# Bernat-C/MRI-Diffusion-SuperResolution

Hardware: AMD Instinct MI355X
Metric: MRI slices/sec (50-step DDIM, 256^2, bs=32) (higher is better)
Workload: dtype bf16; 1 GPU; configs[1]: 256x256 1-ch synthetic MRI slices -> 4x32x32 latents, SD-1.5-size UNet (859.5M params, random init) + rank-4 LoRA, 50-step DDIM, bs=32 per GPU; ddim_steps=50, parallelism=slice-sharded x1 (no collective), lora=explicit adapters, down-projection + rank-r update inside the projection GEMMs, tile_table=profiles/r03_tune_cache.tsv, hipgraph=True

## Files before the change

include/mrisr_debug.h:

```cpp
#ifndef MRISR_DEBUG_H
#define MRISR_DEBUG_H
#ifdef __cplusplus
extern "C" {
#endif

void mrisr_debug_force_split(int splitk);
void mrisr_debug_force_tile(int tile);
void mrisr_debug_prefer_tile(int tile);
void mrisr_debug_gemm_flags(int flags);
void mrisr_debug_gemm_stamps(void* dev_buf, int tile);
void mrisr_debug_group_m(int group_m);
void mrisr_debug_op_conv_pad0(int on);
void mrisr_debug_set_tile_eff(int tile, double eff);
void mrisr_debug_set_tuned(const char* key, int tile, int splitk);
void mrisr_debug_gn_fused(int on);

int mrisr_autotune_stats(int* shapes, double* ms);
void mrisr_autotune_release(void);

int mrisr_bench_gemm(int M, int N, int K, int conv, int B, int H, int W, int stride, int ups, int c1, int tile, int splitk,
                     int iters, float* ms_out);

void mrisr_debug_sk_inkernel(int on);

void mrisr_debug_subpix(int min_rows);

void mrisr_debug_temb_table(int on);

void mrisr_debug_mlp_proj(int on);

void mrisr_debug_gn_slabs(int on);

void mrisr_debug_sc_fused(int on);

void mrisr_debug_ff_proj_fused(int on);

void mrisr_debug_xattn_tail(int on);
void mrisr_debug_xattn_tail_stamps(void* dev_buf);

int mrisr_bench_mlp(int M, int hidden, int iters, float* ms_out);

#ifdef __cplusplus
}
#endif
#endif
```

mri-diffusion-superresolution_amd/csrc/capi_ops.hip:

```cpp
#include <algorithm>
#include <cmath>
#include <cstring>
#include <memory>
#include <vector>

#include "api.h"
#include "model.h"
#include "train_ops.h"

using namespace mrisr;

namespace {
struct OpScratch {
    std::vector<std::unique_ptr<DevBuf>> bufs;
    void* alloc(size_t bytes, bool zero = false) {
        bufs.emplace_back(new DevBuf());
        if (bufs.back()->reserve(bytes ? bytes : 1, zero)) return nullptr;
        return bufs.back()->p;
    }
};
template <typename T>
int op_gemm_run(OpScratch& sc, hipStream_t st, GemmArgs& g) {
    return gemm_run<T>(g, st, false, [&sc](size_t n) { return sc.alloc(n); });
}
// ... 598 lines not shown
    a.x0 = x->data; a.c0 = (int)x->shape[1];
    if (x2) { a.x1 = x2->data; a.c1 = (int)x2->shape[1]; }
    a.B = (int)x->shape[0]; a.HW = (int)(x->shape[2] * x->shape[3]); a.groups = groups; a.eps = eps;
    a.gamma = gamma_dev; a.beta = beta_dev; a.silu = silu; a.y = y->data;
    a.nsplit = groupnorm_nsplit(a.B, a.HW);
    DevBuf part;
    TRY(part.reserve((size_t)a.B * a.nsplit * groups * 2 * sizeof(float), false));
    a.partial = static_cast<float*>(part.p);
    int rc = x->dtype == MRISR_F32 ? launch_groupnorm<float>(a, st) : launch_groupnorm<bf16>(a, st);
    if (rc) return rc;
    MRISR_CHECK_HIP(hipStreamSynchronize(st));
    return 0;
    API_END
}

int mrisr_op_layernorm(const mrisr_tensor* x, const float* gamma_dev, const float* beta_dev, float eps,
                       mrisr_tensor* y, void* stream) {
    API_BEGIN
    TRY(op_dtype_ok(x));
    MRISR_REQUIRE(x->ndim == 2 && y && y->dtype == x->dtype, "rows in/out");
    hipStream_t st = (hipStream_t)stream;
    const int M = (int)x->shape[0], C = (int)x->shape[1];
    return x->dtype == MRISR_F32 ? launch_layernorm<float>(x->data, y->data, gamma_dev, beta_dev, M, C, eps, st)
                                 : launch_layernorm<bf16>(x->data, y->data, gamma_dev, beta_dev, M, C, eps, st);
    API_END
}

int mrisr_op_attention(const mrisr_tensor* q, const mrisr_tensor* k, const mrisr_tensor* v, int heads, int flash,
                       mrisr_tensor* out, void* stream) {
    API_BEGIN
// ... 617 lines not shown
```

mri-diffusion-superresolution_amd/csrc/common.h:

```cpp
#pragma once
#include <hip/hip_runtime.h>
#include <stdint.h>
#include <string>

#include "lora_hr.h"

namespace mrisr {

typedef __bf16 bf16;
typedef __attribute__((ext_vector_type(8))) __bf16 bf16x8;
typedef __attribute__((ext_vector_type(4))) __bf16 bf16x4;
typedef __attribute__((ext_vector_type(4))) float f32x4;
typedef __attribute__((ext_vector_type(16))) float f32x16;

enum DType : int { DT_F32 = 0, DT_BF16 = 1, DT_F16 = 2, DT_I64 = 3 };

template <typename T> struct TypeTag;
template <> struct TypeTag<float> { static constexpr int id = DT_F32; };
template <> struct TypeTag<bf16> { static constexpr int id = DT_BF16; };

__device__ __forceinline__ float to_f32(float x) { return x; }
__device__ __forceinline__ float to_f32(bf16 x) { return (float)x; }
template <typename T> __device__ __forceinline__ T from_f32(float x);
template <> __device__ __forceinline__ float from_f32<float>(float x) { return x; }
// ... 172 lines not shown
    int nsplit = 1;
};
extern int g_plan_salt;
int groupnorm_nsplit(int B, int HW);
struct GnSlabSrc {
    const float* partial = nullptr;
    int splitk = 1;
    float alpha = 1.f;
    const float* bias = nullptr;
    const float* rowvec = nullptr;
    int rowvec_ld = 0, rowvec_div = 1;
    const void* resid = nullptr;
    int ldr = 0;
    void* raw_out = nullptr;
};
bool groupnorm_slabs_ok(int C, int groups, int HW);
int launch_groupnorm_slabs(const GroupNormArgs& a, const GnSlabSrc& s, hipStream_t st);
bool gn_fused_geometry(int c0, int c1, int groups, int HW, int* slab, int* slots, int* rl, int* nv, int ve = 8);
template <typename T> int launch_groupnorm(const GroupNormArgs& a, hipStream_t st);
template <typename T>
int launch_layernorm(const void* x, void* y, const float* gamma, const float* beta, int M, int C, float eps,
                     hipStream_t st);
template <typename T>
int launch_softmax_rows(const float* s, int ld, void* p, int ldp, long long rows, int nk, hipStream_t st);

struct GroupNormBwdArgs {
    const void* x0 = nullptr;
    const void* x1 = nullptr;
    int c0 = 0, c1 = 0, B = 0, HW = 0, groups = 32;
    float eps = 1e-5f;
    const float* gamma = nullptr;
// ... 204 lines not shown
```

mri-diffusion-superresolution_amd/csrc/norm.hip:

```cpp
#include "common.h"
#include "prof.h"

namespace mrisr {

template <typename T> struct Vec;
template <> struct Vec<bf16> {
    static constexpr int N = 8;
    typedef bf16x8 type;
};
template <> struct Vec<float> {
    static constexpr int N = 4;
    typedef f32x4 type;
};

template <typename T, int VPT>
__global__ __launch_bounds__(256) void gn_stats_kernel(const GroupNormArgs a, int slots, int RL) {
    constexpr int VE = Vec<T>::N;
    typedef typename Vec<T>::type vec_t;
    extern __shared__ float sm[];
    const int C = a.c0 + a.c1;
    const int b = blockIdx.y, sp = blockIdx.x;
    const int tid = threadIdx.x;
    const int slot = tid % slots, rl = tid / slots;
    const int rows_per = (a.HW + a.nsplit - 1) / a.nsplit;
// ... 118 lines not shown
            for (int v = 0; v < VPT; ++v) {
                const int ch = (slot * VPT + v) * VE;
                vec_t o;
#pragma unroll
                for (int e = 0; e < VE; ++e) {
                    float f = (float)xv[u][v][e] * sc[v][e] + sh[v][e];
                    if (a.silu) f = silu_f(f);
                    o[e] = from_f32<T>(f);
                }
                *reinterpret_cast<vec_t*>(y + (size_t)r * C + ch) = o;
            }
        }
    }
}

template <int NVM, int VE, bool SLAB = false, int NT = 256>
__global__ __launch_bounds__(NT) void gn_fused_kernel(const GroupNormArgs a, int slab, int slots, int RL, int nslab, int xcd_map, const GnSlabSrc ss = GnSlabSrc()) {
    typedef bf16 T;
    typedef __attribute__((ext_vector_type(VE))) __bf16 vec_t;
    __shared__ float part[NT * 16];
    __shared__ float seg[2 * 1280];
    __shared__ double gsum[2 * 80];
    __shared__ float mean_s[80], rstd_s[80];
    const int C = a.c0 + a.c1;
    const int Cg = C / a.groups;
    int b, sl;
    if (xcd_map) {
        const int L = blockIdx.x;
        b = (L & 7) + 8 * (L / (8 * nslab));
        sl = (L >> 3) % nslab;
    } else {
// ... 2 lines not shown
    }
    const int ch0 = sl * slab;
    const int tid = threadIdx.x;
    const int slot = tid % slots, rl = tid / slots;
    const bool active = rl < RL;
    const int ch = ch0 + slot * VE;
    const T* src;
    int ld;
    if (ch < a.c0) { src = reinterpret_cast<const T*>(a.x0) + (size_t)b * a.HW * a.c0 + ch; ld = a.c0; }
    else { src = reinterpret_cast<const T*>(a.x1) + (size_t)b * a.HW * a.c1 + (ch - a.c0); ld = a.c1; }
    vec_t xv[NVM];
    float s1[VE], s2[VE];
#pragma unroll
    for (int e = 0; e < VE; ++e) s1[e] = s2[e] = 0.f;
    if (active) {
        if constexpr (SLAB) {
            typedef __attribute__((ext_vector_type(VE))) float fvec_t;
            const size_t MN = (size_t)a.B * a.HW * C;
            fvec_t bv;
#pragma unroll
            for (int e = 0; e < VE; ++e) bv[e] = 0.f;
            if (ss.bias) bv = *reinterpret_cast<const fvec_t*>(ss.bias + ch);
#pragma unroll
            for (int i = 0; i < NVM; ++i) {
                const int r = rl + i * RL;
                if (r < a.HW) {
                    const size_t mrow = (size_t)b * a.HW + r;
                    const float* pp = ss.partial + mrow * C + ch;
                    fvec_t v;
#pragma unroll
                    for (int e = 0; e < VE; ++e) v[e] = 0.f;
                    for (int sp = 0; sp < ss.splitk; ++sp) {
                        const fvec_t t = *reinterpret_cast<const fvec_t*>(pp + (size_t)sp * MN);
#pragma unroll
                        for (int e = 0; e < VE; ++e) v[e] += t[e];
                    }
#pragma unroll
                    for (int e = 0; e < VE; ++e) v[e] = v[e] * ss.alpha + bv[e];
                    if (ss.rowvec) {
                        const fvec_t t = *reinterpret_cast<const fvec_t*>(ss.rowvec + (mrow / ss.rowvec_div) * ss.rowvec_ld + ch);
#pragma unroll
                        for (int e = 0; e < VE; ++e) v[e] += t[e];
                    }
                    if (ss.resid) {
                        const vec_t t = *reinterpret_cast<const vec_t*>(reinterpret_cast<const T*>(ss.resid) + mrow * ss.ldr + ch);
#pragma unroll
                        for (int e = 0; e < VE; ++e) v[e] += (float)t[e];
                    }
#pragma unroll
                    for (int e = 0; e < VE; ++e) xv[i][e] = (bf16)v[e];
                    if (ss.raw_out) *reinterpret_cast<vec_t*>(reinterpret_cast<T*>(ss.raw_out) + mrow * C + ch) = xv[i];
                }
            }
        } else {
#pragma unroll
        for (int i = 0; i < NVM; ++i) {
            const int r = rl + i * RL;
            if (r < a.HW) xv[i] = *reinterpret_cast<const vec_t*>(src + (size_t)r * ld);
        }
        }
#pragma unroll
        for (int i = 0; i < NVM; ++i) {
            if (rl + i * RL < a.HW) {
#pragma unroll
                for (int e = 0; e < VE; ++e) {
                    const float f = (float)xv[i][e];
                    s1[e] += f;
// ... 202 lines not shown
    if (rows_per_block < RL) rows_per_block = RL;
    bx = (a.HW + rows_per_block - 1) / rows_per_block;
    ProfScope ps2(prof_intern(n2), 0.0, 2.0 * act_bytes, st);
    switch (vpt) {
        case 1: hipLaunchKernelGGL((gn_apply_kernel<T, 1>), dim3(bx, a.B), dim3(256), 0, st, a, slots, RL, rows_per_block); break;
        case 2: hipLaunchKernelGGL((gn_apply_kernel<T, 2>), dim3(bx, a.B), dim3(256), 0, st, a, slots, RL, rows_per_block); break;
        case 3: hipLaunchKernelGGL((gn_apply_kernel<T, 3>), dim3(bx, a.B), dim3(256), 0, st, a, slots, RL, rows_per_block); break;
        default: hipLaunchKernelGGL((gn_apply_kernel<T, 4>), dim3(bx, a.B), dim3(256), 0, st, a, slots, RL, rows_per_block); break;
    }
    MRISR_CHECK_HIP(hipGetLastError());
    return 0;
}

static int g_gn_slabs = -1;
extern "C" void mrisr_debug_gn_slabs(int on) { g_gn_slabs = on; ++g_plan_salt; }
static bool gn_slabs_geometry(int C, int groups, int HW, int B, int* ve, int* slab, int* slots, int* rl, int* nv) {
    if (!gn_fused_geometry(C, 0, groups, HW, slab, slots, rl, nv, 8)) return false;
    *ve = 8;
    int s4 = 0, sl4 = 0, rl4 = 0, nv4 = 0;
    if (B * (C / *slab) < 512 && gn_fused_geometry(C, 0, groups, HW, &s4, &sl4, &rl4, &nv4, 4) && C / s4 > C / *slab) {
        *ve = 4; *slab = s4; *slots = sl4; *rl = rl4; *nv = nv4;
    }
    return *nv <= 8;
}
bool groupnorm_slabs_ok(int C, int groups, int HW) {
    static const int env = [] { const char* e = getenv("MRISR_GN_SLABS"); return e ? atoi(e) : 1; }();
    if (g_gn_slabs < 0 ? !env : !g_gn_slabs) return false;
    if (C % groups || groups > 64 || C % 8) return false;
    int ve, slab, slots, rl, nv;
    return gn_slabs_geometry(C, groups, HW, 32, &ve, &slab, &slots, &rl, &nv);
}
int launch_groupnorm_slabs(const GroupNormArgs& a, const GnSlabSrc& s, hipStream_t st) {
    const int C = a.c0;
    MRISR_REQUIRE(a.c1 == 0 && a.x1 == nullptr && C % a.groups == 0 && a.groups <= 64 && C % 8 == 0, "GroupNorm from slabs: one source, whole groups");
    MRISR_REQUIRE(s.partial && s.splitk >= 1 && a.partial != nullptr && a.nsplit >= 1 && (!s.rowvec || s.rowvec_div >= 1) && (!s.resid || s.ldr % 8 == 0), "GroupNorm from slabs: operands");
    int ve, slab, slots, rl, nv;
    MRISR_REQUIRE(gn_slabs_geometry(C, a.groups, a.HW, a.B, &ve, &slab, &slots, &rl, &nv), "GroupNorm from slabs: geometry (groupnorm_slabs_ok)");
    const int nslab = C / slab;
    const int xmap = (a.B % 8) == 0 ? 1 : 0;
    std::string nf = "groupnorm_from_slabs";
    if (prof_enabled() && prof_shapes()) {
        char buf[96];
        snprintf(buf, sizeof(buf), " B=%d HW=%d C=%d s=%d", a.B, a.HW, C, s.splitk);
        nf += buf;
    }
    const double act_bytes = (double)a.B * a.HW * C * 2.0;
    ProfScope ps(prof_intern(nf), 0.0, act_bytes * (2.0 * s.splitk + 1.0 + (s.raw_out ? 1.0 : 0.0) + (s.resid ? 1.0 : 0.0)), st);
    const dim3 fg(a.B * nslab);
#define GNS_GO(NV, VEV) hipLaunchKernelGGL((gn_fused_kernel<NV, VEV, true>), fg, dim3(256), 0, st, a, slab, slots, rl, nslab, xmap, s)
    if (ve == 8) { if (nv <= 2) GNS_GO(2, 8); else if (nv <= 4) GNS_GO(4, 8); else GNS_GO(8, 8); }
    else { if (nv <= 2) GNS_GO(2, 4); else if (nv <= 4) GNS_GO(4, 4); else GNS_GO(8, 4); }
#undef GNS_GO
    MRISR_CHECK_HIP(hipGetLastError());
    return 0;
}

__device__ __forceinline__ float wave_sum(float v) {
#pragma unroll
    for (int o = 32; o > 0; o >>= 1) v += __shfl_xor(v, o);
    return v;
}
__device__ __forceinline__ float wave_max(float v) {
#pragma unroll
    for (int o = 32; o > 0; o >>= 1) v = fmaxf(v, __shfl_xor(v, o));
    return v;
}

// ... 241 lines not shown
```

mri-diffusion-superresolution_amd/csrc/runner.h:

```cpp
#pragma once
#include <climits>
#include <cmath>
#include <cstdlib>

#include "api.h"
#include "gemm_args.h"
#include "model.h"

namespace mrisr {

extern int g_subpix_override;

inline bool fuse_ln() {
    static int v = -1;
    if (v < 0) { const char* e = getenv("MRISR_FUSE_LN"); v = (e && e[0] == '0') ? 0 : 1; }
    return v == 1;
}
inline bool lora_in_kernel() {
    static int v = -1;
    if (v < 0) { const char* e = getenv("MRISR_LORA_INKERNEL"); v = (e && e[0] == '0') ? 0 : 1; }
    return v == 1;
}

template <typename T>
// ... 90 lines not shown
        *out = new_act(x.B, x.H, x.W, cw.cout);
        if (!out->p) return 7;
        GroupNormArgs a;
        a.x0 = nullptr; a.c0 = cw.cout; a.B = x.B; a.HW = x.H * x.W; a.groups = m.cfg.norm_num_groups; a.eps = eps;
        a.gamma = nw.g; a.beta = nw.b; a.silu = silu ? 1 : 0; a.y = out->p;
        a.nsplit = groupnorm_nsplit(a.B, a.HW);
        a.partial = static_cast<float*>(alloc((size_t)a.B * a.nsplit * a.groups * 2 * sizeof(float)));
        TRY(gemm_alloc_partial(g, arena_alloc()));
        if (!a.partial) return 7;
        if (dry) return 0;
        g.defer_reduce = 1;
        TRY(launch_gemm<T>(g, st));
        GnSlabSrc ss;
        ss.partial = g.partial; ss.splitk = g.splitk; ss.alpha = g.alpha; ss.bias = g.bias; ss.rowvec = g.rowvec; ss.rowvec_ld = g.rowvec_ld;
        ss.rowvec_div = g.rowvec_div; ss.resid = g.resid; ss.ldr = g.ldr; ss.raw_out = h.p;
        return launch_groupnorm_slabs(a, ss, st);
    }

    static int subpix_min_rows() {
        static const int v = [] { const char* e = getenv("MRISR_SUBPIX"); return e ? atoi(e) : 2048; }();
        return g_subpix_override >= 0 ? g_subpix_override : v;
    }
    int upsample_conv(const Act& x, const Level& lv, Act* out) {
        const int minr = subpix_min_rows();
        if (!(sizeof(T) == 2 && lv.up_sp && !m.keep && minr > 0 && (long long)x.rows() >= minr))
            return conv3(x, nullptr, lv.up, 1, 1, nullptr, 0, 1, nullptr, ACT_NONE, out);
        const ConvW& cw = lv.up;
        MRISR_REQUIRE(cw.cin == x.C, "upsampler weight mismatch");
        *out = new_act(x.B, 2 * x.H, 2 * x.W, cw.cout);
        if (!out->p) return 7;
// ... 93 lines not shown
        TRY(gn(t->h, nullptr, r.n2, true, m.cfg.norm_eps, &t->hn, &t->p2, &t->ns2));
        Act res = x;
        if (r.has_sc) {
            GemmArgs g = resnet_shortcut_args(x, x1, r.sc.w, r.sc.b, r.cin, r.cout, o.p);
            TRY(run_gemm(g));
            res = o;
        } else {
            MRISR_REQUIRE(!x1, "concat input requires a shortcut conv");
        }
        if (r.c2.r) TRY(conv_lora_z(t->hn, r.c2, &t->z2));
        GemmArgs g = resnet_conv2_args(t->hn.p, x.B, x.H, x.W, r.cout, r.c2.w, r.c2.b, res.p, o.p);
        if (t->z2) ga_lora_epilogue(g, r.c2, t->z2);
        return run_gemm(g);
    }

    int resnet(const ResW& r, const Act& x, const Act* x1, Act* out, const NormW* next = nullptr, float next_eps = 0.f, Act* next_out = nullptr) {
        Act o = new_act(x.B, x.H, x.W, r.cout);
        if (!o.p) return 7;
        if (next_out) next_out->p = nullptr;
        if (r.c1.r || r.c2.r) {
            const size_t mk0 = m.arena.mark();
            ResTape t;
            TRY(resnet_literal(r, x, x1, o, &t));
            if (!m.keep) m.arena.release(mk0);
            *out = o;
            return 0;
        }
        GemmArgs g2;
        bool fuse2 = false;
        GroupNormArgs a2;
        GemmArgs gt = resnet_conv2_args(kUnallocated, x.B, x.H, x.W, r.cout, r.c2sc, r.b2sc, nullptr, o.p, r.cin, &x, x1);
        const bool sc_tail = sizeof(T) == 2 && !m.keep && r.has_sc && r.c2sc && sc_fused_enabled() && x.C + (x1 ? x1->C : 0) == r.cin && gemm_sc_tail_ok(gt);
        if (next && next_out && sizeof(T) == 2 && !m.keep && next->c == r.cout && groupnorm_slabs_ok(r.cout, m.cfg.norm_num_groups, x.H * x.W)) {
            g2 = sc_tail ? gt
                         : resnet_conv2_args(kUnallocated, x.B, x.H, x.W, r.cout, r.c2.w, r.c2.b, kUnallocated, kUnallocated);
            TRY(gemm_choose(g2, true));
            fuse2 = g2.splitk > 1;
            if (fuse2) {
                *next_out = new_act(x.B, x.H, x.W, r.cout);
                a2.nsplit = groupnorm_nsplit(x.B, x.H * x.W);
                a2.partial = static_cast<float*>(alloc((size_t)x.B * a2.nsplit * m.cfg.norm_num_groups * 2 * sizeof(float)));
                if (!next_out->p || !a2.partial) return 7;
            }
        }
        const size_t mk = m.arena.mark();
        Act xn, h, hn;
        TRY(gn(x, x1, r.n1, true, m.cfg.norm_eps, &xn));
        const int div = m.t_scalar ? INT_MAX : x.H * x.W;
        TRY(conv3_gn(xn, nullptr, r.c1, m.tproj_out + r.temb_off, m.tproj_total, div, nullptr, r.n2, true, m.cfg.norm_eps, nullptr, &hn));
        Act res = x;
        if (sc_tail) {
            res.p = nullptr;
        } else if (r.has_sc) {
            GemmArgs g = resnet_shortcut_args(x, x1, r.sc.w, r.sc.b, r.cin, r.cout, o.p);
            MRISR_REQUIRE(r.sc.R == 0, "shortcut has no LoRA");
            TRY(run_gemm(g));
            res = o;
        } else {
            MRISR_REQUIRE(!x1, "concat input requires a shortcut conv");
        }
        if (fuse2) {
            g2.a0 = hn.p; g2.resid = res.p; g2.out = o.p;
            TRY(gemm_alloc_partial(g2, arena_alloc()));
            if (!dry) {
                g2.defer_reduce = 1;
                TRY(launch_gemm<T>(g2, st));
                a2.x0 = nullptr; a2.c0 = r.cout; a2.B = x.B; a2.HW = x.H * x.W; a2.groups = m.cfg.norm_num_groups; a2.eps = next_eps;
                a2.gamma = next->g; a2.beta = next->b; a2.silu = 0; a2.y = next_out->p;
                GnSlabSrc ss;
                ss.partial = g2.partial; ss.splitk = g2.splitk; ss.alpha = g2.alpha; ss.bias = g2.bias; ss.resid = res.p; ss.ldr = r.cout; ss.raw_out = o.p;
                TRY(launch_groupnorm_slabs(a2, ss, st));
            }
        } else if (sc_tail) {
            gt.a0 = hn.p;
            TRY(run_gemm(gt));
        } else {
            GemmArgs g = resnet_conv2_args(hn.p, x.B, x.H, x.W, r.cout, r.c2.w, r.c2.b, res.p, o.p);
            TRY(run_gemm(g));
        }
        if (!m.keep) m.arena.release(mk);
        *out = o;
        return 0;
    }
// ... 231 lines not shown
            MRISR_CHECK_HIP(hipMemcpyAsync(t.data, a.p, a.numel() * sizeof(T), hipMemcpyDeviceToDevice, st));
            return 0;
        }
        return launch_nhwc_to_nchw<T>(a.p, t.data, t.dtype, a.B, a.C, a.H, a.W, scale, st);
    }
    int add_external(Act& x, const mrisr_tensor& t) {
        const size_t mk = m.arena.mark();
        Act r;
        TRY(import_act(t, &r, false));
        MRISR_REQUIRE(r.B == x.B && r.C == x.C && r.H == x.H && r.W == x.W, "residual shape mismatch");
        if (!dry) TRY(launch_add_inplace<T>(x.p, r.p, (long long)x.numel(), st));
        if (!m.keep) m.arena.release(mk);
        return 0;
    }

    int encoder(Act x, const mrisr_tensor* intrablock, int n_intra, std::vector<Act>* skips, Act* out, int last_skip = -1) {
        skips->push_back(x);
        int ib = 0;
        auto done = [&] { return last_skip >= 0 && (int)skips->size() > last_skip; };
        for (int i = 0; i < m.cfg.num_levels && !done(); ++i) {
            Level& lv = m.down[i];
            const bool has_attn = !lv.xf.empty();
            const int block_last = (int)skips->size() - 1 + (int)lv.res.size() + (lv.has_down ? 1 : 0);
            for (size_t j = 0; j < lv.res.size() && !done(); ++j) {
                Act y, xn_next;
                xn_next.p = nullptr;
                if (has_attn) TRY(resnet(lv.res[j], x, nullptr, &y, &lv.xf[j].norm, 1e-6f, &xn_next));
                else TRY(resnet(lv.res[j], x, nullptr, &y));
                x = y;
                if (has_attn) {
                    TRY(transformer(lv.xf[j], x, &y, &xn_next));
                    x = y;
                    if (j + 1 == lv.res.size() && ib < n_intra) TRY(add_external(x, intrablock[ib++]));
                }
                skips->push_back(x);
            }
            if (lv.has_down && !done()) {
                Act y;
                TRY(conv3(x, nullptr, lv.down, 2, 0, nullptr, 0, 1, nullptr, ACT_NONE, &y));
                x = y;
                skips->push_back(x);
            }
            if (!has_attn && ib < n_intra && (last_skip < 0 || last_skip >= block_last)) {
                TRY(add_external(x, intrablock[ib++]));
            }
        }
        *out = x;
        return 0;
    }
    int mid(Act x, Act* out) {
        Act y, xn_next;
        xn_next.p = nullptr;
        TRY(resnet(m.mid_r0, x, nullptr, &y, &m.mid_xf.norm, 1e-6f, &xn_next));
        x = y;
        TRY(transformer(m.mid_xf, x, &y, &xn_next));
        x = y;
        TRY(resnet(m.mid_r1, x, nullptr, &y));
        *out = y;
        return 0;
    }

    int set_context(const mrisr_tensor& ehs) {
        MRISR_REQUIRE(ehs.ndim == 3 && ehs.shape[2] == m.cfg.cross_attention_dim, "encoder_hidden_states shape");
        MRISR_REQUIRE((int)ehs.shape[0] == m.ws_B && (int)ehs.shape[1] == m.ctx_len, "context shape vs planned workspace");
        if (!dry) TRY(launch_nchw_to_nhwc<T>(ehs.data, ehs.dtype, m.ctx_rows, m.ws_B * m.ctx_len, m.cfg.cross_attention_dim, 1, 1, st));
        auto each = [&](XfW& x) -> int { return project_context(x, m.head_buf_for_C(x.C)); };
        for (auto& lv : m.down) for (auto& x : lv.xf) TRY(each(x));
        TRY(each(m.mid_xf));
// ... 16 lines not shown
        m.arena.reset();
        const int B = (int)sample.shape[0];
        const bool store = fc.mode == CACHE_STORE, use = fc.mode == CACHE_USE;
        const int q0 = m.num_skips() - 1 - fc.depth;
        if (store || use) {
            MRISR_REQUIRE(q0 >= 0 && fc.depth >= 1 && fc.p, "feature cache: depth 1 .. num_skips - 1 and a buffer");
            MRISR_REQUIRE(n_down == 0 && !mid_res, "a feature cache together with ControlNet residuals is not supported");
        }
        if (ehs) TRY(set_context(*ehs));
        MRISR_REQUIRE(dry || m.ctx_valid, "no encoder_hidden_states given and none cached");
        TRY(time_embed(t_dev, t_scalar, B));
        Act s, x;
        TRY(import_act(sample, &s, false));
        TRY(direct(s, m.conv_in, 1, ACT_NONE, nullptr, &x));
        std::vector<Act> skips;
        TRY(encoder(x, intrablock, n_intra, &skips, &x, use ? fc.depth : -1));
        if (n_down > 0) {
            MRISR_REQUIRE(n_down == (int)skips.size(), "down_block_additional_residuals count");
            for (int k = 0; k < n_down; ++k) {
                if (skips[k].p == x.p) {
                    Act c = new_act(x.B, x.H, x.W, x.C);
                    if (!c.p) return 7;
                    if (!dry) MRISR_CHECK_HIP(hipMemcpyAsync(c.p, x.p, x.numel() * sizeof(T), hipMemcpyDeviceToDevice, st));
                    skips[k] = c;
                }
                TRY(add_external(skips[k], down_res[k]));
            }
        }
        if (!use) TRY(mid(x, &x));
        if (mid_res) TRY(add_external(x, *mid_res));
        int q = 0;
        for (int i = 0; i < m.cfg.num_levels; ++i) {
            Level& lv = m.up[i];
            for (size_t j = 0; j < lv.res.size(); ++j, ++q) {
                if (use && q < q0) continue;
                if ((store || use) && q == q0) {
                    int64_t cs[4];
                    TRY(m.cache_shape(fc.depth, B, (int)sample.shape[2], (int)sample.shape[3], cs));
                    if (store) {
                        MRISR_REQUIRE(x.B == cs[0] && x.C == cs[1] && x.H == cs[2] && x.W == cs[3], "feature cache shape");
                        if (!dry) MRISR_CHECK_HIP(hipMemcpyAsync(fc.p, x.p, x.numel() * sizeof(T), hipMemcpyDeviceToDevice, st));
                    } else {
                        x.p = fc.p; x.B = (int)cs[0]; x.C = (int)cs[1]; x.H = (int)cs[2]; x.W = (int)cs[3];
                    }
// ... 46 lines not shown
    int controlnet_forward(const mrisr_tensor& sample, const long long* t_dev, int t_scalar, const mrisr_tensor* ehs,
                           const mrisr_tensor* cond, float scale, mrisr_tensor* down_out, int n_down,
                           mrisr_tensor* mid_out) {
        m.arena.reset();
        const int B = (int)sample.shape[0];
        if (ehs) TRY(set_context(*ehs));
        if (cond) TRY(set_cond(*cond));
        MRISR_REQUIRE(dry || (m.ctx_valid && m.cond_valid), "context / condition image neither given nor cached");
        TRY(time_embed(t_dev, t_scalar, B));
        Act s, x;
        TRY(import_act(sample, &s, false));
        Act ce;
        ce.p = m.cond_emb; ce.B = B; ce.H = s.H; ce.W = s.W; ce.C = m.cfg.block_out_channels[0];
        TRY(direct(s, m.conv_in, 1, ACT_NONE, &ce, &x));
        std::vector<Act> skips;
        TRY(encoder(x, nullptr, 0, &skips, &x));
        TRY(mid(x, &x));
        MRISR_REQUIRE(n_down == (int)skips.size(), "ControlNet output count");
        for (int k = 0; k < n_down; ++k) {
            const size_t mk = m.arena.mark();
            Act o = new_act(skips[k].B, skips[k].H, skips[k].W, skips[k].C);
            if (!o.p) return 7;
            TRY(linear(skips[k].p, (int)skips[k].rows(), skips[k].C, m.cn_down[k], ACT_NONE, nullptr, 0, nullptr, o.p, o.C));
            TRY(export_act(o, down_out[k], scale));
            if (!m.keep) m.arena.release(mk);
        }
        Act o = new_act(x.B, x.H, x.W, x.C);
        if (!o.p) return 7;
        TRY(linear(x.p, (int)x.rows(), x.C, m.cn_mid, ACT_NONE, nullptr, 0, nullptr, o.p, o.C));
        return export_act(o, *mid_out, scale);
    }
};
// ... 3 lines not shown
```

mri-diffusion-superresolution_amd/mrisr/_lib.py:

```python
from __future__ import annotations

import ctypes as C
import os
from typing import Optional, Sequence

import torch

_HERE = os.path.dirname(os.path.abspath(__file__))
LIB_PATH = os.path.join(os.path.dirname(_HERE), "csrc", "libmrisr.so")

MRISR_F32, MRISR_BF16, MRISR_F16, MRISR_I64 = 0, 1, 2, 3
MRISR_NCHW, MRISR_NHWC = 0, 1
STEP_DDIM, STEP_RESSHIFT, STEP_DDPM, STEP_UNIPC, STEP_DPMSOLVERPP = 0, 1, 2, 3, 4
ACT_NONE, ACT_RELU, ACT_SILU, ACT_GEGLU = 0, 1, 2, 3
TILE_WINDOWS = {"uniform": 0, "gaussian": 1}

_DT = {torch.float32: MRISR_F32, torch.bfloat16: MRISR_BF16, torch.float16: MRISR_F16, torch.int64: MRISR_I64}


class Tensor(C.Structure):
    _fields_ = [("data", C.c_void_p), ("dtype", C.c_int32), ("layout", C.c_int32), ("ndim", C.c_int32),
                ("shape", C.c_int64 * 4)]


# ... 72 lines not shown
        L.mrisr_sampler_destroy.restype = None
        L.mrisr_sampler_set_clip.argtypes = [C.c_void_p, C.c_float]
        L.mrisr_sampler_set_guidance.argtypes = [C.c_void_p, C.c_float, C.c_float]
        L.mrisr_op_guided_step.argtypes = [C.c_int, C.c_void_p, C.c_void_p, C.c_void_p, C.c_void_p, C.c_void_p, C.c_void_p, C.c_float,
                                           C.c_float, C.c_float, C.c_void_p]
        L.mrisr_sampler_set_cache.argtypes = [C.c_void_p, C.c_int, C.c_int]
        L.mrisr_unet_cache_shape.argtypes = [C.c_void_p, C.c_int, C.c_int, C.c_int, C.c_int, C.c_void_p]
        L.mrisr_unet_forward_cached.argtypes = [C.c_void_p, C.c_void_p, C.c_void_p, C.c_void_p, C.c_void_p, C.c_int, C.c_int, C.c_int,
                                                C.c_void_p, C.c_void_p, C.c_void_p]
        L.mrisr_sampler_set_solver.argtypes = [C.c_void_p, C.c_int, C.c_int, C.c_int, C.c_void_p, C.c_int]
        L.mrisr_op_multistep_step.argtypes = [C.c_int, C.c_void_p, C.c_void_p, C.c_void_p, C.c_void_p, C.c_void_p, C.c_void_p, C.c_void_p,
                                              C.c_int, C.c_int, C.c_float, C.c_float, C.c_void_p]
        P, I, F, Q = C.c_void_p, C.c_int, C.c_float, C.c_int64
        L.mrisr_op_groupnorm_bwd.argtypes = [I, P, I, P, I, I, I, P, P, I, F, I, P, P, I, P, I, P, P, P]
        L.mrisr_op_layernorm_bwd.argtypes = [I, P, P, P, P, I, I, F, I, P, P, P]
        L.mrisr_op_geglu.argtypes = [I, I, P, P, P, Q, I, P]
        L.mrisr_op_pointwise_bwd.argtypes = [I, I, P, P, P, P, Q, I, I, I, I, I, I, I, P]
        L.mrisr_op_lora_wgrad.argtypes = [I, P, I, P, I, I, I, I, I, I, I, P, P, P, F, P]
        L.mrisr_op_lora_wgrad_geglu.argtypes = [I, P, I, P, I, I, I, I, P, F, P]
        L.mrisr_op_lora_wgrad_hr.argtypes = [I, P, I, P, I, I, I, I, I, I, I, P, P, P, F, I, P]
        L.mrisr_op_dora_scale.argtypes = [I, P, P, P, P, F, P, P, I, I, I, I, I, I, P]
        L.mrisr_op_dora_mag_grad.argtypes = [I, P, I, P, I, P, I, P, P, P, I, I, I, P]
        L.mrisr_model_set_dora.argtypes = [P, I]
        L.mrisr_op_transpose.argtypes = [I, P, P, I, I, I, I, Q, Q, I, I, P]
        L.mrisr_op_softmax_bwd.argtypes = [I, P, P, P, I, Q, I, F, P]
        L.mrisr_op_small_dense_bwd.argtypes = [I, I, P, I, P, I, I, I, I, I, P, I, P, P, I, P]
        L.mrisr_op_conv_wgrad.argtypes = [I, P, I, I, I, I, P, I, I, I, I, I, P, P, I, I, I, P]
        L.mrisr_op_conv_dgrad.argtypes = [I, P, I, I, I, I, P, I, I, P, I, P]
        L.mrisr_op_conv_lora_down.argtypes = [I, P, I, I, I, I, P, I, P, I, P]
        L.mrisr_op_conv_lora_dgrad.argtypes = [I, P, I, I, I, I, P, I, P, I, P]
# ... 88 lines not shown
```

mri-diffusion-superresolution_amd/mrisr/ops.py:

```python
from __future__ import annotations

import ctypes as C
from typing import Optional

import torch

from . import _lib as L


def _nhwc(x: torch.Tensor):
    buf = x.permute(0, 2, 3, 1).contiguous()
    return buf, L.as_tensor(buf, L.MRISR_NHWC, shape=x.shape)


def _f32(x: Optional[torch.Tensor]):
    return None if x is None else C.c_void_p(x.detach().to(torch.float32).contiguous().data_ptr())


def conv3x3(x, weight, bias=None, x2=None, stride=1, upsample=False, act=L.ACT_NONE, splitk=0, tile=0, subpix=False):
    xb, tx = _nhwc(x)
    t2 = None
    if x2 is not None:
        x2b, t2 = _nhwc(x2)
    w = weight.detach().to(torch.float32).contiguous()
# ... 144 lines not shown
    ctot = x.shape[1]
    if x2 is not None:
        x2b, t2 = _nhwc(x2)
        ctot += x2.shape[1]
    g = gamma.detach().to(torch.float32).contiguous()
    b = beta.detach().to(torch.float32).contiguous()
    B, _, H, W = x.shape
    yb = torch.empty((B, H, W, ctot), dtype=x.dtype, device=x.device)
    ty = L.as_tensor(yb, L.MRISR_NHWC, shape=(B, ctot, H, W))
    L.check(L.lib().mrisr_op_groupnorm(C.byref(tx), C.byref(t2) if t2 else None, C.c_void_p(g.data_ptr()),
                                       C.c_void_p(b.data_ptr()), groups, C.c_float(eps), 1 if silu else 0,
                                       C.byref(ty), L.stream_ptr()))
    return yb.permute(0, 3, 1, 2)


def layernorm(x, gamma, beta, eps=1e-5):
    x = x.contiguous()
    g = gamma.detach().to(torch.float32).contiguous()
    b = beta.detach().to(torch.float32).contiguous()
    y = torch.empty_like(x)
    tx, ty = L.as_tensor(x), L.as_tensor(y)
    L.check(L.lib().mrisr_op_layernorm(C.byref(tx), C.c_void_p(g.data_ptr()), C.c_void_p(b.data_ptr()), C.c_float(eps),
                                       C.byref(ty), L.stream_ptr()))
    torch.cuda.current_stream().synchronize()
    return y


def attention(q, k, v, heads, flash=True, fp8=False):
    q, k, v = q.contiguous(), k.contiguous(), v.contiguous()
    out = torch.empty_like(q)
# ... 179 lines not shown
```

Baseline: 72.54 slices/s.

## Fuse split-K reduce with next GroupNorm in encoder downsample and resnet chains

Adds a conv3_down path in which the stride-2 downsample conv defers its split-K reduction into the GroupNorm-from-slabs kernel of the next resnet's first norm (with SiLU). Resnet outputs in non-attention encoder levels now also produce the next block's normalized input, which is passed forward as a precomputed `pre` activation so the following resnet skips its own GroupNorm. The slab kernel gains a split-K-specialized variant that batches partial-slab loads across rows, and it accepts a second concatenated source. This removes separate reduce and norm passes over activations, at the cost of more template instantiations and more complex encoder control flow.

```diff
diff --git a/include/mrisr_debug.h b/include/mrisr_debug.h
--- a/include/mrisr_debug.h
+++ b/include/mrisr_debug.h
@@ -31,6 +31,10 @@
 
 void mrisr_debug_gn_slabs(int on);
 
+int mrisr_op_groupnorm_slabs(const float* slabs, int splitk, int B, int HW, int C, const float* bias, const float* rowvec, int rowvec_ld,
+                             int rowvec_div, const void* resid, int ldr, const void* x1, int c1, const float* gamma_dev, const float* beta_dev,
+                             int groups, float eps, int silu, int merged, void* y, void* raw, int* merged_out, void* stream);
+
 void mrisr_debug_sc_fused(int on);
 
 void mrisr_debug_ff_proj_fused(int on);
diff --git a/mri-diffusion-superresolution_amd/csrc/capi_ops.hip b/mri-diffusion-superresolution_amd/csrc/capi_ops.hip
--- a/mri-diffusion-superresolution_amd/csrc/capi_ops.hip
+++ b/mri-diffusion-superresolution_amd/csrc/capi_ops.hip
@@ -636,6 +636,43 @@
     API_END
 }
 
+int mrisr_op_groupnorm_slabs(const float* slabs, int splitk, int B, int HW, int C, const float* bias, const float* rowvec, int rowvec_ld,
+                             int rowvec_div, const void* resid, int ldr, const void* x1, int c1, const float* gamma_dev, const float* beta_dev,
+                             int groups, float eps, int silu, int merged, void* y, void* raw, int* merged_out, void* stream) {
+    API_BEGIN
+    MRISR_REQUIRE(slabs && splitk >= 1 && B >= 1 && HW >= 1 && C >= 8 && C % 8 == 0 && gamma_dev && beta_dev && y, "GroupNorm from slabs: operands");
+    MRISR_REQUIRE((c1 == 0) == (x1 == nullptr) && c1 % 8 == 0 && (C + c1) % groups == 0 && groups <= 64, "GroupNorm from slabs: second source, groups");
+    MRISR_REQUIRE((!rowvec || (rowvec_div >= 1 && rowvec_ld >= C)) && (!resid || (ldr >= C && ldr % 8 == 0)), "GroupNorm from slabs: time row / residual pitch");
+    hipStream_t st = (hipStream_t)stream;
+    GroupNormArgs a;
+    a.B = B; a.HW = HW; a.groups = groups; a.eps = eps; a.gamma = gamma_dev; a.beta = beta_dev; a.silu = silu; a.y = y;
+    a.nsplit = groupnorm_nsplit(B, HW);
+    DevBuf part, tmp;
+    TRY(part.reserve((size_t)B * a.nsplit * groups * 2 * sizeof(float), false));
+    a.partial = static_cast<float*>(part.p);
+    const bool go = merged && groupnorm_slabs_ok(C, groups, HW, c1, B);
+    if (merged_out) *merged_out = go ? 1 : 0;
+    if (go) {
+        a.x0 = nullptr; a.c0 = C; a.x1 = x1; a.c1 = c1;
+        GnSlabSrc ss;
+        ss.partial = slabs; ss.splitk = splitk; ss.bias = bias; ss.rowvec = rowvec; ss.rowvec_ld = rowvec_ld; ss.rowvec_div = rowvec_div;
+        ss.resid = resid; ss.ldr = ldr; ss.raw_out = raw;
+        TRY(launch_groupnorm_slabs(a, ss, st));
+    } else {
+        void* h = raw;
+        if (!h) { TRY(tmp.reserve((size_t)B * HW * C * sizeof(bf16), false)); h = tmp.p; }
+        GemmArgs g;
+        g.M = B * HW; g.N = C; g.splitk = splitk; g.partial = const_cast<float*>(slabs); g.bias = bias;
+        ga_rowvec(g, rowvec, rowvec_ld, rowvec_div); ga_resid(g, resid, ldr); ga_out(g, h, C);
+        TRY(launch_splitk_reduce<bf16>(g, st));
+        a.x0 = h; a.c0 = C; a.x1 = x1; a.c1 = c1;
+        TRY(launch_groupnorm<bf16>(a, st));
+    }
+    MRISR_CHECK_HIP(hipStreamSynchronize(st));
+    return 0;
+    API_END
+}
+
 int mrisr_op_layernorm(const mrisr_tensor* x, const float* gamma_dev, const float* beta_dev, float eps,
                        mrisr_tensor* y, void* stream) {
     API_BEGIN
diff --git a/mri-diffusion-superresolution_amd/csrc/common.h b/mri-diffusion-superresolution_amd/csrc/common.h
--- a/mri-diffusion-superresolution_amd/csrc/common.h
+++ b/mri-diffusion-superresolution_amd/csrc/common.h
@@ -210,7 +210,7 @@
     int ldr = 0;
     void* raw_out = nullptr;
 };
-bool groupnorm_slabs_ok(int C, int groups, int HW);
+bool groupnorm_slabs_ok(int C, int groups, int HW, int c1 = 0, int B = 32);
 int launch_groupnorm_slabs(const GroupNormArgs& a, const GnSlabSrc& s, hipStream_t st);
 bool gn_fused_geometry(int c0, int c1, int groups, int HW, int* slab, int* slots, int* rl, int* nv, int ve = 8);
 template <typename T> int launch_groupnorm(const GroupNormArgs& a, hipStream_t st);
diff --git a/mri-diffusion-superresolution_amd/csrc/norm.hip b/mri-diffusion-superresolution_amd/csrc/norm.hip
--- a/mri-diffusion-superresolution_amd/csrc/norm.hip
+++ b/mri-diffusion-superresolution_amd/csrc/norm.hip
@@ -156,7 +156,7 @@
     }
 }
 
-template <int NVM, int VE, bool SLAB = false, int NT = 256>
+template <int NVM, int VE, bool SLAB = false, int NT = 256, int SK = 0>
 __global__ __launch_bounds__(NT) void gn_fused_kernel(const GroupNormArgs a, int slab, int slots, int RL, int nslab, int xcd_map, const GnSlabSrc ss = GnSlabSrc()) {
     typedef bf16 T;
     typedef __attribute__((ext_vector_type(VE))) __bf16 vec_t;
@@ -189,19 +189,83 @@
 #pragma unroll
     for (int e = 0; e < VE; ++e) s1[e] = s2[e] = 0.f;
     if (active) {
-        if constexpr (SLAB) {
+        if (SLAB && ch0 < a.c0) {
             typedef __attribute__((ext_vector_type(VE))) float fvec_t;
-            const size_t MN = (size_t)a.B * a.HW * C;
+            const int Cs = a.c0;
+            const size_t MN = (size_t)a.B * a.HW * Cs;
             fvec_t bv;
 #pragma unroll
             for (int e = 0; e < VE; ++e) bv[e] = 0.f;
             if (ss.bias) bv = *reinterpret_cast<const fvec_t*>(ss.bias + ch);
+            if constexpr (SK > 0) {
+                constexpr int BUD = 32, CSMAX = VE == 4 ? 16 : 4;
+                constexpr int CS = SK <= CSMAX ? SK : CSMAX;
+                constexpr int RB0 = BUD / (CS * VE), RB = RB0 < 1 ? 1 : (RB0 > NVM ? NVM : RB0);
+                static_assert(NVM % RB == 0 && SK % CS == 0, "row batches and split chunks divide evenly");
+#pragma unroll
+                for (int i0 = 0; i0 < NVM; i0 += RB) {
+                    size_t mrow[RB];
+                    fvec_t tv[RB], t[RB][CS];
+                    vec_t rs[RB];
+#pragma unroll
+                    for (int u = 0; u < RB; ++u) mrow[u] = (size_t)b * a.HW + min(rl + (i0 + u) * RL, a.HW - 1);
+                    if (ss.rowvec) {
+#pragma unroll
+                        for (int u = 0; u < RB; ++u) tv[u] = *reinterpret_cast<const fvec_t*>(ss.rowvec + (mrow[u] / ss.rowvec_div) * ss.rowvec_ld + ch);
+                    }
+                    if (ss.resid) {
+#pragma unroll
+                        for (int u = 0; u < RB; ++u) rs[u] = *reinterpret_cast<const vec_t*>(reinterpret_cast<const T*>(ss.resid) + mrow[u] * ss.ldr + ch);
+                    }
+#pragma unroll
+                    for (int u = 0; u < RB; ++u)
+#pragma unroll
+                        for (int sp = 0; sp < CS; ++sp) t[u][sp] = *reinterpret_cast<const fvec_t*>(ss.partial + (size_t)sp * MN + mrow[u] * Cs + ch);
+#pragma unroll
+                    for (int u = 0; u < RB; ++u) {
+                        fvec_t v;
+#pragma unroll
+                        for (int e = 0; e < VE; ++e) v[e] = 0.f;
+#pragma unroll
+                        for (int sp = 0; sp < CS; ++sp)
+#pragma unroll
+                            for (int e = 0; e < VE; ++e) v[e] += t[u][sp][e];
+#pragma unroll
+                        for (int c = CS; c < SK; c += CS) {
+#pragma unroll
+                            for (int sp = 0; sp < CS; ++sp) t[u][sp] = *reinterpret_cast<const fvec_t*>(ss.partial + (size_t)(c + sp) * MN + mrow[u] * Cs + ch);
+#pragma unroll
+                            for (int sp = 0; sp < CS; ++sp)
+#pragma unroll
+                                for (int e = 0; e < VE; ++e) v[e] += t[u][sp][e];
+                        }
+                        if (ss.bias) {
+#pragma unroll
+                            for (int e = 0; e < VE; ++e) v[e] = v[e] * ss.alpha + bv[e];
+                        } else {
+#pragma unroll
+                            for (int e = 0; e < VE; ++e) v[e] = v[e] * ss.alpha + 0.f;
+                        }
+                        if (ss.rowvec) {
+#pragma unroll
+                            for (int e = 0; e < VE; ++e) v[e] += tv[u][e];
+                        }
+                        if (ss.resid) {
+#pragma unroll
+                            for (int e = 0; e < VE; ++e) v[e] += (float)rs[u][e];
+                        }
+#pragma unroll
+                        for (int e = 0; e < VE; ++e) xv[i0 + u][e] = (bf16)v[e];
+                        if (ss.raw_out && rl + (i0 + u) * RL < a.HW) *reinterpret_cast<vec_t*>(reinterpret_cast<T*>(ss.raw_out) + mrow[u] * Cs + ch) = xv[i0 + u];
+                    }
+                }
+            } else {
 #pragma unroll
             for (int i = 0; i < NVM; ++i) {
                 const int r = rl + i * RL;
                 if (r < a.HW) {
                     const size_t mrow = (size_t)b * a.HW + r;
-                    const float* pp = ss.partial + mrow * C + ch;
+                    const float* pp = ss.partial + mrow * Cs + ch;
                     fvec_t v;
 #pragma unroll
                     for (int e = 0; e < VE; ++e) v[e] = 0.f;
@@ -224,8 +288,9 @@
                     }
 #pragma unroll
                     for (int e = 0; e < VE; ++e) xv[i][e] = (bf16)v[e];
-                    if (ss.raw_out) *reinterpret_cast<vec_t*>(reinterpret_cast<T*>(ss.raw_out) + mrow * C + ch) = xv[i];
+                    if (ss.raw_out) *reinterpret_cast<vec_t*>(reinterpret_cast<T*>(ss.raw_out) + mrow * Cs + ch) = xv[i];
                 }
+            }
             }
         } else {
 #pragma unroll
@@ -458,28 +523,30 @@
 
 static int g_gn_slabs = -1;
 extern "C" void mrisr_debug_gn_slabs(int on) { g_gn_slabs = on; ++g_plan_salt; }
-static bool gn_slabs_geometry(int C, int groups, int HW, int B, int* ve, int* slab, int* slots, int* rl, int* nv) {
-    if (!gn_fused_geometry(C, 0, groups, HW, slab, slots, rl, nv, 8)) return false;
+static bool gn_slabs_geometry(int c0, int c1, int groups, int HW, int B, int* ve, int* slab, int* slots, int* rl, int* nv) {
+    const int C = c0 + c1;
+    if (!gn_fused_geometry(c0, c1, groups, HW, slab, slots, rl, nv, 8)) return false;
     *ve = 8;
     int s4 = 0, sl4 = 0, rl4 = 0, nv4 = 0;
-    if (B * (C / *slab) < 512 && gn_fused_geometry(C, 0, groups, HW, &s4, &sl4, &rl4, &nv4, 4) && C / s4 > C / *slab) {
+    if (B * (C / *slab) < 512 && gn_fused_geometry(c0, c1, groups, HW, &s4, &sl4, &rl4, &nv4, 4) && C / s4 > C / *slab) {
         *ve = 4; *slab = s4; *slots = sl4; *rl = rl4; *nv = nv4;
     }
+    if (c0 % *slab) return false;
     return *nv <= 8;
 }
-bool groupnorm_slabs_ok(int C, int groups, int HW) {
+bool groupnorm_slabs_ok(int C, int groups, int HW, int c1, int B) {
     static const int env = [] { const char* e = getenv("MRISR_GN_SLABS"); return e ? atoi(e) : 1; }();
     if (g_gn_slabs < 0 ? !env : !g_gn_slabs) return false;
-    if (C % groups || groups > 64 || C % 8) return false;
+    if ((C + c1) % groups || groups > 64 || C % 8 || c1 % 8) return false;
     int ve, slab, slots, rl, nv;
-    return gn_slabs_geometry(C, groups, HW, 32, &ve, &slab, &slots, &rl, &nv);
+    return gn_slabs_geometry(C, c1, groups, HW, B, &ve, &slab, &slots, &rl, &nv);
 }
 int launch_groupnorm_slabs(const GroupNormArgs& a, const GnSlabSrc& s, hipStream_t st) {
-    const int C = a.c0;
-    MRISR_REQUIRE(a.c1 == 0 && a.x1 == nullptr && C % a.groups == 0 && a.groups <= 64 && C % 8 == 0, "GroupNorm from slabs: one source, whole groups");
+    const int C = a.c0 + a.c1;
+    MRISR_REQUIRE((a.c1 == 0) == (a.x1 == nullptr) && C % a.groups == 0 && a.groups <= 64 && a.c0 % 8 == 0 && a.c1 % 8 == 0, "GroupNorm from slabs: whole groups, a second source with its width");
     MRISR_REQUIRE(s.partial && s.splitk >= 1 && a.partial != nullptr && a.nsplit >= 1 && (!s.rowvec || s.rowvec_div >= 1) && (!s.resid || s.ldr % 8 == 0), "GroupNorm from slabs: operands");
     int ve, slab, slots, rl, nv;
-    MRISR_REQUIRE(gn_slabs_geometry(C, a.groups, a.HW, a.B, &ve, &slab, &slots, &rl, &nv), "GroupNorm from slabs: geometry (groupnorm_slabs_ok)");
+    MRISR_REQUIRE(gn_slabs_geometry(a.c0, a.c1, a.groups, a.HW, a.B, &ve, &slab, &slots, &rl, &nv), "GroupNorm from slabs: geometry (groupnorm_slabs_ok)");
     const int nslab = C / slab;
     const int xmap = (a.B % 8) == 0 ? 1 : 0;
     std::string nf = "groupnorm_from_slabs";
@@ -488,13 +555,22 @@
         snprintf(buf, sizeof(buf), " B=%d HW=%d C=%d s=%d", a.B, a.HW, C, s.splitk);
         nf += buf;
     }
-    const double act_bytes = (double)a.B * a.HW * C * 2.0;
-    ProfScope ps(prof_intern(nf), 0.0, act_bytes * (2.0 * s.splitk + 1.0 + (s.raw_out ? 1.0 : 0.0) + (s.resid ? 1.0 : 0.0)), st);
+    const double act_bytes = (double)a.B * a.HW * a.c0 * 2.0;
+    ProfScope ps(prof_intern(nf), 0.0, act_bytes * (2.0 * s.splitk + 1.0 + (s.raw_out ? 1.0 : 0.0) + (s.resid ? 1.0 : 0.0)) + 4.0 * a.B * a.HW * a.c1, st);
     const dim3 fg(a.B * nslab);
-#define GNS_GO(NV, VEV) hipLaunchKernelGGL((gn_fused_kernel<NV, VEV, true>), fg, dim3(256), 0, st, a, slab, slots, rl, nslab, xmap, s)
-    if (ve == 8) { if (nv <= 2) GNS_GO(2, 8); else if (nv <= 4) GNS_GO(4, 8); else GNS_GO(8, 8); }
-    else { if (nv <= 2) GNS_GO(2, 4); else if (nv <= 4) GNS_GO(4, 4); else GNS_GO(8, 4); }
-#undef GNS_GO
+#define GNS_SK(NV, VEV, SKV) hipLaunchKernelGGL((gn_fused_kernel<NV, VEV, true, 256, SKV>), fg, dim3(256), 0, st, a, slab, slots, rl, nslab, xmap, s)
+#define GNS_GO4(NV)                                                                                                          \
+    switch (s.splitk) {                                                                                                      \
+        case 2: GNS_SK(NV, 4, 2); break;                                                                                     \
+        case 4: GNS_SK(NV, 4, 4); break;                                                                                     \
+        case 8: GNS_SK(NV, 4, 8); break;                                                                                     \
+        case 16: GNS_SK(NV, 4, 16); break;                                                                                   \
+        default: GNS_SK(NV, 4, 0); break;                                            \
+    }
+    if (ve == 8) { if (nv <= 2) GNS_SK(2, 8, 0); else if (nv <= 4) GNS_SK(4, 8, 0); else GNS_SK(8, 8, 0); }
+    else { if (nv <= 2) GNS_GO4(2) else if (nv <= 4) GNS_GO4(4) else GNS_GO4(8) }
+#undef GNS_GO4
+#undef GNS_SK
     MRISR_CHECK_HIP(hipGetLastError());
     return 0;
 }
diff --git a/mri-diffusion-superresolution_amd/csrc/runner.h b/mri-diffusion-superresolution_amd/csrc/runner.h
--- a/mri-diffusion-superresolution_amd/csrc/runner.h
+++ b/mri-diffusion-superresolution_amd/csrc/runner.h
@@ -128,6 +128,35 @@
         GnSlabSrc ss;
         ss.partial = g.partial; ss.splitk = g.splitk; ss.alpha = g.alpha; ss.bias = g.bias; ss.rowvec = g.rowvec; ss.rowvec_ld = g.rowvec_ld;
         ss.rowvec_div = g.rowvec_div; ss.resid = g.resid; ss.ldr = g.ldr; ss.raw_out = h.p;
+        return launch_groupnorm_slabs(a, ss, st);
+    }
+
+    int conv3_down(const Act& x, const ConvW& cw, const NormW* next, float next_eps, Act* out, Act* next_out) {
+        next_out->p = nullptr;
+        MRISR_REQUIRE(cw.cin == x.C && cw.ks == 3, "conv3x3 weight mismatch");
+        GemmArgs g = conv3_args(x, nullptr, cw, 2, 0, nullptr, 0, 1, nullptr, ACT_NONE);
+        bool fuse = next && sizeof(T) == 2 && !m.keep && next->c == cw.cout && groupnorm_slabs_ok(cw.cout, m.cfg.norm_num_groups, g.Hout * g.Wout);
+        if (fuse) {
+            g.out = kUnallocated;
+            TRY(gemm_choose(g, true));
+            fuse = g.splitk > 1;
+        }
+        if (!fuse) return conv3(x, nullptr, cw, 2, 0, nullptr, 0, 1, nullptr, ACT_NONE, out);
+        *out = new_act(x.B, g.Hout, g.Wout, cw.cout);
+        *next_out = new_act(x.B, g.Hout, g.Wout, cw.cout);
+        GroupNormArgs a;
+        a.x0 = nullptr; a.c0 = cw.cout; a.B = x.B; a.HW = g.Hout * g.Wout; a.groups = m.cfg.norm_num_groups; a.eps = next_eps;
+        a.gamma = next->g; a.beta = next->b; a.silu = 1; a.y = next_out->p;
+        a.nsplit = groupnorm_nsplit(a.B, a.HW);
+        a.partial = static_cast<float*>(alloc((size_t)a.B * a.nsplit * a.groups * 2 * sizeof(float)));
+        TRY(gemm_alloc_partial(g, arena_alloc()));
+        if (!out->p || !next_out->p || !a.partial) return 7;
+        if (dry) return 0;
+        g.out = out->p;
+        g.defer_reduce = 1;
+        TRY(launch_gemm<T>(g, st));
+        GnSlabSrc ss;
+        ss.partial = g.partial; ss.splitk = g.splitk; ss.alpha = g.alpha; ss.bias = g.bias; ss.raw_out = out->p;
         return launch_groupnorm_slabs(a, ss, st);
     }
 
@@ -251,7 +280,8 @@
         return run_gemm(g);
     }
 
-    int resnet(const ResW& r, const Act& x, const Act* x1, Act* out, const NormW* next = nullptr, float next_eps = 0.f, Act* next_out = nullptr) {
+    int resnet(const ResW& r, const Act& x, const Act* x1, Act* out, const NormW* next = nullptr, float next_eps = 0.f, Act* next_out = nullptr,
+               bool next_silu = false, const Act* pre = nullptr) {
         Act o = new_act(x.B, x.H, x.W, r.cout);
         if (!o.p) return 7;
         if (next_out) next_out->p = nullptr;
@@ -282,7 +312,8 @@
         }
         const size_t mk = m.arena.mark();
         Act xn, h, hn;
-        TRY(gn(x, x1, r.n1, true, m.cfg.norm_eps, &xn));
+        if (pre && pre->p) xn = *pre;
+        else TRY(gn(x, x1, r.n1, true, m.cfg.norm_eps, &xn));
         const int div = m.t_scalar ? INT_MAX : x.H * x.W;
         TRY(conv3_gn(xn, nullptr, r.c1, m.tproj_out + r.temb_off, m.tproj_total, div, nullptr, r.n2, true, m.cfg.norm_eps, nullptr, &hn));
         Act res = x;
@@ -303,7 +334,7 @@
                 g2.defer_reduce = 1;
                 TRY(launch_gemm<T>(g2, st));
                 a2.x0 = nullptr; a2.c0 = r.cout; a2.B = x.B; a2.HW = x.H * x.W; a2.groups = m.cfg.norm_num_groups; a2.eps = next_eps;
-                a2.gamma = next->g; a2.beta = next->b; a2.silu = 0; a2.y = next_out->p;
+                a2.gamma = next->g; a2.beta = next->b; a2.silu = next_silu ? 1 : 0; a2.y = next_out->p;
                 GnSlabSrc ss;
                 ss.partial = g2.partial; ss.splitk = g2.splitk; ss.alpha = g2.alpha; ss.bias = g2.bias; ss.resid = res.p; ss.ldr = r.cout; ss.raw_out = o.p;
                 TRY(launch_groupnorm_slabs(a2, ss, st));
@@ -565,10 +596,13 @@
         return 0;
     }
 
-    int encoder(Act x, const mrisr_tensor* intrablock, int n_intra, std::vector<Act>* skips, Act* out, int last_skip = -1) {
+    int encoder(Act x, const mrisr_tensor* intrablock, int n_intra, std::vector<Act>* skips, Act* out, int last_skip = -1, Act* out_pre = nullptr) {
         skips->push_back(x);
         int ib = 0;
         auto done = [&] { return last_skip >= 0 && (int)skips->size() > last_skip; };
+        Act pend;
+        pend.p = nullptr;
+        auto n1_of = [&](const ResW& r) -> const NormW* { return (dry || n_intra == 0) && last_skip < 0 && !(r.c1.r || r.c2.r) ? &r.n1 : nullptr; };
         for (int i = 0; i < m.cfg.num_levels && !done(); ++i) {
             Level& lv = m.down[i];
             const bool has_attn = !lv.xf.empty();
@@ -576,8 +610,14 @@
             for (size_t j = 0; j < lv.res.size() && !done(); ++j) {
                 Act y, xn_next;
                 xn_next.p = nullptr;
-                if (has_attn) TRY(resnet(lv.res[j], x, nullptr, &y, &lv.xf[j].norm, 1e-6f, &xn_next));
-                else TRY(resnet(lv.res[j], x, nullptr, &y));
+                const Act pre = pend;
+                pend.p = nullptr;
+                if (has_attn) {
+                    TRY(resnet(lv.res[j], x, nullptr, &y, &lv.xf[j].norm, 1e-6f, &xn_next, false, &pre));
+                } else {
+                    const NormW* nx = j + 1 < lv.res.size() ? n1_of(lv.res[j + 1]) : (!lv.has_down && i + 1 == m.cfg.num_levels ? n1_of(m.mid_r0) : nullptr);
+                    TRY(resnet(lv.res[j], x, nullptr, &y, nx, m.cfg.norm_eps, &pend, true, &pre));
+                }
                 x = y;
                 if (has_attn) {
                     TRY(transformer(lv.xf[j], x, &y, &xn_next));
@@ -588,7 +628,7 @@
             }
             if (lv.has_down && !done()) {
                 Act y;
-                TRY(conv3(x, nullptr, lv.down, 2, 0, nullptr, 0, 1, nullptr, ACT_NONE, &y));
+                TRY(conv3_down(x, lv.down, i + 1 < m.cfg.num_levels ? n1_of(m.down[i + 1].res[0]) : nullptr, m.cfg.norm_eps, &y, &pend));
                 x = y;
                 skips->push_back(x);
             }
@@ -597,12 +637,13 @@
             }
         }
         *out = x;
-        return 0;
-    }
-    int mid(Act x, Act* out) {
+        if (out_pre) *out_pre = pend;
+        return 0;
+    }
+    int mid(Act x, Act* out, const Act* pre = nullptr) {
         Act y, xn_next;
         xn_next.p = nullptr;
-        TRY(resnet(m.mid_r0, x, nullptr, &y, &m.mid_xf.norm, 1e-6f, &xn_next));
+        TRY(resnet(m.mid_r0, x, nullptr, &y, &m.mid_xf.norm, 1e-6f, &xn_next, false, pre));
         x = y;
         TRY(transformer(m.mid_xf, x, &y, &xn_next));
         x = y;
@@ -649,7 +690,9 @@
         TRY(import_act(sample, &s, false));
         TRY(direct(s, m.conv_in, 1, ACT_NONE, nullptr, &x));
         std::vector<Act> skips;
-        TRY(encoder(x, intrablock, n_intra, &skips, &x, use ? fc.depth : -1));
+        Act mid_pre;
+        mid_pre.p = nullptr;
+        TRY(encoder(x, intrablock, n_intra, &skips, &x, use ? fc.depth : -1, &mid_pre));
         if (n_down > 0) {
             MRISR_REQUIRE(n_down == (int)skips.size(), "down_block_additional_residuals count");
             for (int k = 0; k < n_down; ++k) {
@@ -662,7 +705,7 @@
                 TRY(add_external(skips[k], down_res[k]));
             }
         }
-        if (!use) TRY(mid(x, &x));
+        if (!use) TRY(mid(x, &x, &mid_pre));
         if (mid_res) TRY(add_external(x, *mid_res));
         int q = 0;
         for (int i = 0; i < m.cfg.num_levels; ++i) {
@@ -739,8 +782,10 @@
         ce.p = m.cond_emb; ce.B = B; ce.H = s.H; ce.W = s.W; ce.C = m.cfg.block_out_channels[0];
         TRY(direct(s, m.conv_in, 1, ACT_NONE, &ce, &x));
         std::vector<Act> skips;
-        TRY(encoder(x, nullptr, 0, &skips, &x));
-        TRY(mid(x, &x));
+        Act mid_pre;
+        mid_pre.p = nullptr;
+        TRY(encoder(x, nullptr, 0, &skips, &x, -1, &mid_pre));
+        TRY(mid(x, &x, &mid_pre));
         MRISR_REQUIRE(n_down == (int)skips.size(), "ControlNet output count");
         for (int k = 0; k < n_down; ++k) {
             const size_t mk = m.arena.mark();
diff --git a/mri-diffusion-superresolution_amd/mrisr/_lib.py b/mri-diffusion-superresolution_amd/mrisr/_lib.py
--- a/mri-diffusion-superresolution_amd/mrisr/_lib.py
+++ b/mri-diffusion-superresolution_amd/mrisr/_lib.py
@@ -110,6 +110,7 @@
         P, I, F, Q = C.c_void_p, C.c_int, C.c_float, C.c_int64
         L.mrisr_op_groupnorm_bwd.argtypes = [I, P, I, P, I, I, I, P, P, I, F, I, P, P, I, P, I, P, P, P]
         L.mrisr_op_layernorm_bwd.argtypes = [I, P, P, P, P, I, I, F, I, P, P, P]
+        L.mrisr_op_groupnorm_slabs.argtypes = [P, I, I, I, I, P, P, I, I, P, I, P, I, P, P, I, F, I, I, P, P, P, P]
         L.mrisr_op_geglu.argtypes = [I, I, P, P, P, Q, I, P]
         L.mrisr_op_pointwise_bwd.argtypes = [I, I, P, P, P, P, Q, I, I, I, I, I, I, I, P]
         L.mrisr_op_lora_wgrad.argtypes = [I, P, I, P, I, I, I, I, I, I, I, P, P, P, F, P]
diff --git a/mri-diffusion-superresolution_amd/mrisr/ops.py b/mri-diffusion-superresolution_amd/mrisr/ops.py
--- a/mri-diffusion-superresolution_amd/mrisr/ops.py
+++ b/mri-diffusion-superresolution_amd/mrisr/ops.py
@@ -182,6 +182,22 @@
     return yb.permute(0, 3, 1, 2)
 
 
+def groupnorm_slabs(slabs, B, HW, gamma, beta, y, raw=None, bias=None, rowvec=None, rowvec_div=1, resid=None, x1=None, groups=32, eps=1e-5,
+                    silu=False, merged=True):
+    S, M, Cc = slabs.shape
+    assert M == B * HW and slabs.dtype == torch.float32 and slabs.is_contiguous() and y.is_contiguous()
+    p = lambda a: C.c_void_p(a.data_ptr()) if a is not None else None
+    for t in (raw, x1):
+        assert t is None or (t.is_contiguous() and t.dtype == torch.bfloat16)
+    assert resid is None or (resid.stride(1) == 1 and resid.dtype == torch.bfloat16)
+    ran = C.c_int(-1)
+    L.check(L.lib().mrisr_op_groupnorm_slabs(p(slabs), S, B, HW, Cc, p(bias), p(rowvec), rowvec.stride(0) if rowvec is not None else 0,
+                                             rowvec_div, p(resid), resid.stride(0) if resid is not None else 0, p(x1),
+                                             x1.shape[1] if x1 is not None else 0, p(gamma), p(beta), groups, C.c_float(eps),
+                                             1 if silu else 0, 1 if merged else 0, p(y), p(raw), C.byref(ran), L.stream_ptr()))
+    return ran.value == 1
+
+
 def layernorm(x, gamma, beta, eps=1e-5):
     x = x.contiguous()
     g = gamma.detach().to(torch.float32).contiguous()
```

Result: no change. 72.98 slices/s, median of 5 (+0.6%).
